# hmatuschek/libsdr

Measured on NVIDIA B200. Metric: iq_msamples_per_s_iqbaseband_fmdemod, higher is better.
Workload: dtype f32

## Files before the change

libsdr_b200/csrc/api.cu:

```cuda
#include "iqbb_kernels.cuh"

#include <atomic>
#include <cstdarg>
#include <cstdio>
#include <cmath>
#include <cstring>
#include <map>
#include <mutex>
#include <vector>

namespace sdrg {

static thread_local char g_err[512] = "";
static thread_local int g_device = 0;
static std::atomic<uint64_t> g_launches{0};

int set_error(int code, const char *fmt, ...) {
  va_list ap;
  va_start(ap, fmt);
  vsnprintf(g_err, sizeof(g_err), fmt, ap);
  va_end(ap);
  return code;
}
void count_launch(unsigned n) { g_launches.fetch_add(n, std::memory_order_relaxed); }
// ... 53 lines not shown

}

using namespace sdrg;

struct sdrg_iqbb {
  IqbbDesign d;
  int device = 0;
  bool configured = false;
  double nco_Fs = 0;
  void *d_taps = nullptr, *d_lut = nullptr;
  void *d_hist[2] = {nullptr, nullptr};
  void *d_acc[2] = {nullptr, nullptr};
  size_t acc_cap = 0;
  uint32_t acc_dirty[2] = {0, 0};
  uint32_t taps_len = 1, hist_len = 0;
  std::vector<int32_t> host_taps;
  int in_fmt = 0;
  bool real_input = false;
  double r_Ff = 0, r_width = 0, r_Fs = 0;
  int float_path = 0;
  bool fold = false;
  void *d_tab_a = nullptr, *d_tab_u = nullptr;
  void *d_tab_v = nullptr, *d_tab_cls = nullptr;
  uint32_t v_rows = 0, v_pitch = 0;
  int last_float_kernel = 0;
  uint32_t *d_work = nullptr;
  uint32_t phase0 = 0;
  int parity = 0;
  uint64_t consumed = 0, produced = 0;
// ... 174 lines not shown
int ensure_acc(sdrg_iqbb *h, size_t slots) {
  if (h->acc_cap >= slots) return SDRG_OK;
  const size_t cap = slots + slots / 2 + 64;
  void *n0 = nullptr, *n1 = nullptr;
  SDRG_CUDA(cudaMalloc(&n0, cap * acc_bytes()));
  SDRG_CUDA(cudaMalloc(&n1, cap * acc_bytes()));
  SDRG_CUDA(cudaMemset(n0, 0, cap * acc_bytes()));
  SDRG_CUDA(cudaMemset(n1, 0, cap * acc_bytes()));
  if (h->d_acc[0]) {
    SDRG_CUDA(cudaDeviceSynchronize());
    SDRG_CUDA(cudaMemcpy(h->parity == 0 ? n0 : n1, h->d_acc[h->parity], 2 * acc_bytes(), cudaMemcpyDeviceToDevice));
    cudaFree(h->d_acc[0]); cudaFree(h->d_acc[1]);
  }
  h->d_acc[0] = n0; h->d_acc[1] = n1;
  h->acc_dirty[0] = h->acc_dirty[1] = 0;
  h->acc_cap = cap;
  return SDRG_OK;
}

void reset_stream_state(sdrg_iqbb *h) {
  h->phase0 = 0; h->consumed = 0; h->produced = 0;
}

int design_only(sdrg_iqbb *h) {
  IqbbDesign &d = h->d;
  if (d.oFs > 0 && !h->real_input) {
    d.sub_sample = size_t(d.Fs / d.oFs);
    if (d.sub_sample < 1) d.sub_sample = 1;
  }
  if (d.sub_sample < 1) d.sub_sample = 1;
// ... 33 lines not shown
  const Advance adv = advance(h, n);
  *n_out = adv.n_out;
  int rc = ensure_acc(h, adv.n_out + 3);
  if (rc) return rc;
  const int p = h->parity, q = p ^ 1;
  IqbbAccumArgs a{};
  a.x = d_in; a.hist_in = h->d_hist[p]; a.hist_out = h->d_hist[q];
  a.taps = h->d_taps; a.lut = h->d_lut;
  a.host_taps = (h->d.scalar != SDRG_T_F32 && !h->host_taps.empty()) ? h->host_taps.data() : nullptr;
  a.acc_cur = h->d_acc[p]; a.acc_next = h->d_acc[q];
  a.n = n; a.taps_len = h->taps_len; a.hist_len = h->hist_len;
  a.ss = (uint32_t)h->d.sub_sample; a.r0 = adv.r0; a.first = adv.first;
  a.phase0 = h->phase0; a.inc = (uint32_t)(h->d.lut_inc & 0x7fffu); a.nco = h->d.lut_inc != 0 ? 1u : 0u;
  a.neg = h->d.negative ? 1u : 0u;
  a.zero_next = h->acc_dirty[q];
  a.in_fmt = (uint32_t)h->in_fmt;
  a.fir_shift = h->real_input ? (h->d.scalar == SDRG_T_S8 ? 8u : 16u) : 14u;
  IqbbFinalizeArgs f{};
  f.acc_cur = h->d_acc[p]; f.acc_next = h->d_acc[q];
  f.bb_out = d_bb; f.audio_out = d_audio;
  f.fm_last_in = fm_last_in; f.fm_last_out = fm_last_out;
  f.n_out = (uint32_t)adv.n_out; f.ss = a.ss; f.demod = (uint32_t)demod; f.e0 = adv.e0;
  f.seg = seg; f.in_place = (uint32_t)in_place;
  f.narrow16 = (h->real_input && h->d.scalar == SDRG_T_S8) ? 1u : 0u;
  if (h->fold) {
    IqbbFoldArgs fa{};
    fa.x = d_in; fa.acc_cur = a.acc_cur; fa.acc_next = a.acc_next;
    fa.tab_a = (const float2 *)h->d_tab_a; fa.tab_u = (const float2 *)h->d_tab_u;
    fa.tab_v = (const float2 *)h->d_tab_v; fa.tab_cls = (const uint16_t *)h->d_tab_cls;
    fa.v_rows = h->v_rows; fa.v_pitch = h->v_pitch;
    fa.n = n; fa.taps_len = (uint32_t)h->d.order; fa.ss = a.ss; fa.r0 = a.r0; fa.first = a.first;
    fa.phase0 = a.nco ? a.phase0 : 0u; fa.inc = a.nco ? a.inc : 0u;
    fa.zero_next = a.zero_next; fa.variant = h->float_path == 3 ? 2u : 0u;
    fa.work = h->d_work; f.work_reset = h->d_work;
    ProfScope ps(SDRG_KERNEL_IQBB_ACCUM, st);
    rc = launch_iqbb_fold(fa, st, &h->last_float_kernel);
  } else {
    ProfScope ps(SDRG_KERNEL_IQBB_ACCUM, st);
    if (h->d.scalar == SDRG_T_F32) h->last_float_kernel = 1;
    rc = launch_iqbb_accum(h->d.scalar, a, st);
  }
  if (rc) return rc;
  {
    ProfScope ps(SDRG_KERNEL_IQBB_FINALIZE, st);
    rc = launch_iqbb_finalize(h->d.scalar, f, st);
  }
  if (rc) return rc;
  h->acc_dirty[p] = (uint32_t)adv.n_out + 2;
  h->acc_dirty[q] = 2;
  h->parity = q;
  h->phase0 = (uint32_t)((h->phase0 + (uint64_t)n * (h->d.lut_inc & 0x7fffu)) & 0x7fffu);
  h->consumed += n; h->produced += adv.n_out;
  return SDRG_OK;
}

int check_handle(const sdrg_iqbb *h) {
  if (!h) return set_error(SDRG_ERR_ARG, "IQBaseBand: null handle");
  if (!h->configured) return set_error(SDRG_ERR_RUNTIME, "IQBaseBand: process() before config()");
  return SDRG_OK;
}

int config_common(const char *who, int expect_type, const sdrg_config *src, bool need_rate, bool *skip) {
  *skip = false;
  if (!src) return set_error(SDRG_ERR_ARG, "%s: null config", who);
// ... 287 lines not shown
  h->real_input = true; h->in_fmt = scalar == SDRG_T_S8 ? 5 : 4;
  h->r_Ff = Ff; h->r_width = width;
  return SDRG_OK;
}

int sdrg_iqbb_destroy(sdrg_iqbb *h) {
  if (!h) return SDRG_OK;
  cudaSetDevice(h->device);
  if (h->stream) { cudaStreamSynchronize(h->stream); cudaStreamDestroy(h->stream); }
  else cudaDeviceSynchronize();
  free_dev(&h->d_taps); free_dev(&h->d_lut);
  free_dev(&h->d_hist[0]); free_dev(&h->d_hist[1]);
  free_dev(&h->d_acc[0]); free_dev(&h->d_acc[1]);
  free_dev(&h->d_tab_a); free_dev(&h->d_tab_u); free_dev(&h->d_tab_v); free_dev(&h->d_tab_cls);
  if (h->d_work) { cudaFree(h->d_work); h->d_work = nullptr; }
  free_dev(&h->d_in); free_dev(&h->d_out);
  delete h;
  return SDRG_OK;
}

static int refresh_kernel(sdrg_iqbb *h) {
  if (!h->configured) return SDRG_OK;
  SDRG_CUDA(cudaSetDevice(h->device));
  SDRG_CUDA(cudaDeviceSynchronize());
  const uint32_t old_hist = h->hist_len;
  design_filter(h);
  std::vector<char> keep;
  const size_t sb = in_sample_bytes(h);
  if (old_hist) { keep.resize(old_hist * sb); SDRG_CUDA(cudaMemcpy(keep.data(), h->d_hist[h->parity], keep.size(), cudaMemcpyDeviceToHost)); }
  int rc = upload_design(h);
// ... 597 lines not shown
```

libsdr_b200/csrc/iqbb_finalize.cuh:

```cuda
#pragma once
#include "iqbb_kernels.cuh"
#include "demod_math.cuh"

namespace sdrg {

template <int SCALAR> struct Fin;
template <> struct Fin<SDRG_T_S16> {
  typedef int2 Acc; typedef short2 Bb; typedef short Fm; typedef short Au; typedef int Last;
  static __device__ __forceinline__ int2 value(const Acc s, uint32_t ss) {
    if (ss == 1) return make_int2((int)(short)s.x, (int)(short)s.y);
    return make_int2((int)(short)cdiv_component(s.x, (int)ss), (int)(short)cdiv_component(s.y, (int)ss));
  }
  static __device__ __forceinline__ Bb store(int2 v) { return make_short2((short)v.x, (short)v.y); }
  static __device__ __forceinline__ Last phi(int2 v) { return fm_phi_int(v.x, v.y); }
  static __device__ __forceinline__ Fm fm(Last last, Last p) { return (short)(last - p); }
  static __device__ __forceinline__ Fm fm_first(int2 v) { return (short)v.x; }
  static __device__ __forceinline__ Au am(int2 v) { return (short)am_int(v.x, v.y); }
  static __device__ __forceinline__ Au usb(int2 v) { return (short)usb_int(v.x, v.y); }
};
template <> struct Fin<SDRG_T_S8> {
  typedef int2 Acc; typedef char2 Bb; typedef short Fm; typedef signed char Au; typedef int Last;
  static __device__ __forceinline__ int2 value(const Acc s, uint32_t ss) {
    if (ss == 1) return make_int2((int)(signed char)s.x, (int)(signed char)s.y);
    return make_int2((int)(signed char)cdiv_component(s.x, (int)ss), (int)(signed char)cdiv_component(s.y, (int)ss));
// ... 32 lines not shown
}
template <int SCALAR>
__device__ __forceinline__ auto fin_value(const typename Fin<SCALAR>::Acc s, const IqbbFinalizeArgs &a) {
  if constexpr (SCALAR == SDRG_T_S8) { if (a.narrow16) return fin_value_s8_real(s, a.ss); }
  return Fin<SCALAR>::value(s, a.ss);
}

__device__ __forceinline__ bool seg_first(uint32_t j, const IqbbFinalizeArgs &a) {
  if (j == 0) return true;
  if (a.seg == 0) return false;
  const uint32_t e = a.e0 + j * a.ss;
  return (e % (uint32_t)a.seg) < a.ss;
}

template <int SCALAR>
__device__ __forceinline__ void iqbb_finalize_block(const IqbbFinalizeArgs &a, const uint32_t j0, const int tid,
                                                    typename Fin<SCALAR>::Last *sphi, unsigned char *sskip) {
  typedef Fin<SCALAR> F;
  const typename F::Acc *acc = (const typename F::Acc *)a.acc_cur;
  const uint32_t j = j0 + tid;
  const bool fm = a.demod == SDRG_DEMOD_FM;
  if (j == 0) {
    if (a.work_reset) *a.work_reset = 0u;
    ((typename F::Acc *)a.acc_next)[0] = acc[a.n_out];
    ((typename F::Acc *)a.acc_next)[1] = acc[a.n_out + 1];
    if (fm) {
      typename F::Last last = *(const typename F::Last *)a.fm_last_in;
      for (int64_t k = (int64_t)a.n_out - 1; k >= 0; --k) {
        if (!seg_first((uint32_t)k, a)) { last = F::phi(fin_value<SCALAR>(acc[k], a)); break; }
      }
      *(typename F::Last *)a.fm_last_out = last;
    }
  }
  const bool valid = j < a.n_out;
  auto v = fin_value<SCALAR>(valid ? acc[j] : typename F::Acc(), a);
  if (valid && a.bb_out) ((typename F::Bb *)a.bb_out)[j] = F::store(v);
  if (!a.audio_out) return;
  if (a.demod == SDRG_DEMOD_AM) { if (valid) ((typename F::Au *)a.audio_out)[j] = F::am(v); return; }
  if (a.demod == SDRG_DEMOD_USB) { if (valid) ((typename F::Au *)a.audio_out)[j] = F::usb(v); return; }
  if (!fm) return;
  const bool skip = !valid || seg_first(j, a);
  const typename F::Last p = skip ? typename F::Last(0) : F::phi(v);
  sphi[tid] = p; sskip[tid] = skip ? 1 : 0;
  __syncthreads();
  if (!valid) return;
  typename F::Fm *out = (typename F::Fm *)a.audio_out;
  if (skip) { if (a.in_place) out[j] = F::fm_first(v); return; }
  typename F::Last last;
  if (tid > 0 && !sskip[tid - 1]) last = sphi[tid - 1];
  else {
    int64_t k = (int64_t)j - 1;
    while (k >= 0 && seg_first((uint32_t)k, a)) --k;
    last = (k >= 0) ? F::phi(fin_value<SCALAR>(acc[k], a)) : *(const typename F::Last *)a.fm_last_in;
  }
  out[j] = F::fm(last, p);
}

}
```

libsdr_b200/csrc/iqbb_fold_kernels.cu:

```cuda
#include "iqbb_fold_common.cuh"

namespace sdrg {
using namespace foldk;
namespace {

template <int RS>
__device__ __forceinline__ void ragged_batch(float2 (&R)[8], const float2 *__restrict__ xk, uint32_t ph, uint32_t inc32,
                                             const float2 *sA, bool last_ok) {
  float2 xv[RS];
#pragma unroll
  for (int u = 0; u + 1 < RS; ++u) xv[u] = ld_stream(xk + 32 * u);
  xv[RS - 1] = make_float2(0.f, 0.f);
  if (last_ok) xv[RS - 1] = ld_stream(xk + 32 * (RS - 1));
#pragma unroll
  for (int u = 0; u < RS; ++u) cfma(R[u], sA[((ph + u * inc32) & 0x7fffu) >> 8], xv[u]);
}

__global__ void __launch_bounds__(kFoldThreads, 4) iqbb_fold_f32_kernel(const IqbbFoldArgs a) {
  extern __shared__ __align__(16) unsigned char dyn_smem[];
  __shared__ float2 sA[128];
  __shared__ float2 sH[256];
  const int tid = threadIdx.x, lane = tid & 31, warp = tid >> 5;

  for (uint32_t k = blockIdx.x * blockDim.x + tid; k < a.zero_next; k += gridDim.x * blockDim.x)
// ... 53 lines not shown
      cfma(sent, cmul(Ab, ut0), xt0);
      cfma(sent, cmul(Ab, ut1), xt1);
      float2 tot = make_float2(-sent.x, -sent.y);
#pragma unroll
      for (int u = 0; u < 8; ++u) cfma(tot, sH[(r0 + u * inc32) & 255u], R[u]);
      stage.push(tot, id, lane, acc_out);
      if (L1 > 0) stage.push(sent, id + 1, lane, acc_out);
      continue;
    }
    fold_chunk_general(a, id, total_warps, x, sA, sH, lane, L1, win_off, inc32, inc256, stage, acc_out);
  }
  stage.drain(lane, acc_out);

}

template <int S, int P = 0, int TS = 3>
__global__ void __launch_bounds__(kFoldThreads, S <= 8 ? 4 : (S <= 13 ? 3 : 2)) iqbb_fold_f32_win_kernel(const IqbbFoldArgs a) {
  extern __shared__ __align__(16) unsigned char dyn_smem[];
  __shared__ float2 sA[128];
  __shared__ float2 sH[256];
  const int tid = threadIdx.x, lane = tid & 31, warp = tid >> 5;
  for (uint32_t k = blockIdx.x * blockDim.x + tid; k < a.zero_next; k += gridDim.x * blockDim.x)
    ((float2 *)a.acc_next)[k] = make_float2(0.f, 0.f);
  if (tid < 128) sA[tid] = a.tab_a[tid];
  sH[tid] = a.tab_u[(size_t)tid * a.taps_len];
  __syncthreads();

  const uint32_t T = gridDim.x * kFoldWarps;
  const uint32_t wg = warp * gridDim.x + blockIdx.x;
  const float2 *__restrict__ x = (const float2 *)a.x;
  float *acc_out = (float *)a.acc_cur;
  WarpStage stage{(float2 *)dyn_smem + (size_t)warp * kStageRows * kStagePitch, 0u, 0u};
  const int L1 = (int)a.taps_len - 1;
  const int win_off = (int)a.first - (int)a.r0;
  const uint32_t inc32 = (32u * a.inc) & 0x7fffu, inc256 = (256u * a.inc) & 0x7fffu;
  const bool last_ok = (uint32_t)lane < a.fast_pl;
  int te[TS]; bool te_ok[TS];
#pragma unroll
  for (int k = 0; k < TS; ++k) { te[k] = (int)a.ss - 32 * (S - 1 - k) - lane; te_ok[k] = te[k] >= 1 && te[k] <= L1; }

  if (wg == 0) fold_chunk_general(a, 0u, T, x, sA, sH, lane, L1, win_off, inc32, inc256, stage, acc_out);
  else if (a.fast_hi + wg < a.n_chunks) fold_chunk_general(a, a.fast_hi + wg, T, x, sA, sH, lane, L1, win_off, inc32, inc256, stage, acc_out);
  const uint32_t kWorkChunk = a.work_chunk;
  const uint32_t n_work = (a.fast_hi + kWorkChunk - 1) / kWorkChunk;
  uint32_t grabbed = 0;
  if (lane == 0) grabbed = atomicAdd(a.work, 1u);
  const uint32_t c0 = __shfl_sync(kFull, grabbed, 0);
  if (c0 < n_work) {
    uint32_t id = 1 + c0 * kWorkChunk, end = min(id + kWorkChunk, a.fast_hi + 1);
    if (lane == 0) grabbed = atomicAdd(a.work, 1u);
    const float2 *__restrict__ xc = x + ((int)(id * a.ss) + win_off) + lane;
    float2 ring[S];
#pragma unroll
    for (int i = 0; i + 1 < S; ++i) ring[i] = ld_stream(xc + 32 * i);
    ring[S - 1] = make_float2(0.f, 0.f);
    if (last_ok) ring[S - 1] = ld_stream(xc + 32 * (S - 1));
    float2 carry = make_float2(0.f, 0.f);
    for (;;) {
      uint32_t nid = id + 1;
      bool more = nid < end, switched = false;
      if (!more) {
        const uint32_t cn = __shfl_sync(kFull, grabbed, 0);
        if (cn < n_work) { nid = 1 + cn * kWorkChunk; more = true; switched = true; }
      }
// ... 20 lines not shown
        if (!(P & 1) && S - 1 - i < TS) cfma(ts, ut[S - 1 - i], ring[i]);
        if (more) {
          if (i + 1 < S) ring[i] = ld_stream(xn + 32 * i);
          else if (last_ok) ring[i] = ld_stream(xn + 32 * i);
        }
      }
      const float2 sent = cmul(Ab, ts);
      float2 tot = make_float2(-sent.x, -sent.y);
      const uint32_t r0 = ph & 255u;
#pragma unroll
      for (int u = 0; u < 8; ++u) {
        if (P & 4) { tot.x += R[u].x; tot.y += R[u].y; }
        else cfma(tot, sH[(r0 + u * inc32) & 255u], R[u]);
      }
      tot.x += carry.x; tot.y += carry.y;
      stage.push(tot, id, lane, acc_out);
      carry = sent;
      if ((!more || switched) && L1 > 0 && !(P & 1)) { stage.push(carry, id + 1, lane, acc_out); carry = make_float2(0.f, 0.f); }
      if (!more) break;
      if (switched) {
        end = min(nid + kWorkChunk, a.fast_hi + 1);
        if (lane == 0) grabbed = atomicAdd(a.work, 1u);
      }
      id = nid;
    }
  }
  stage.drain(lane, acc_out);
}

template <int S, int P = 0, int TS = 3>
static int launch_fold_win_s(const IqbbFoldArgs &a, cudaStream_t st) {
  static std::atomic<int> resident_dev[kMaxDevices];
  const size_t smem = (size_t)kFoldWarps * kStageRows * kStagePitch * sizeof(float2);
  const int dev = current_device();
  if (!resident_dev[dev]) {
    SDRG_CUDA(cudaFuncSetAttribute(iqbb_fold_f32_win_kernel<S, P, TS>, cudaFuncAttributeMaxDynamicSharedMemorySize, (int)smem));
    int sms = 0, per_sm = 0;
    SDRG_CUDA(cudaDeviceGetAttribute(&sms, cudaDevAttrMultiProcessorCount, dev));
    SDRG_CUDA(cudaOccupancyMaxActiveBlocksPerMultiprocessor(&per_sm, iqbb_fold_f32_win_kernel<S, P, TS>, kFoldThreads, smem));
    resident_dev[dev] = sms * (per_sm > 0 ? per_sm : 1);
  }
  const uint64_t resident = (uint64_t)resident_dev[dev];
  const uint64_t want = ((uint64_t)a.n_chunks + kFoldWarps - 1) / kFoldWarps;
  iqbb_fold_f32_win_kernel<S, P, TS><<<(unsigned)(want < resident ? want : resident), kFoldThreads, smem, st>>>(a);
  SDRG_CHECK_LAUNCH("iqbb_fold_f32_win_kernel");
  return SDRG_OK;
}

static int launch_fold_win(const IqbbFoldArgs &a, cudaStream_t st) {
#ifdef SDRG_EXPERIMENTS
  static const int wp = env_int("SDRG_FOLD_WINP", 0);
  if (wp && (a.ss + 31) / 32 == 13) {
    switch (wp) {
      case 1: return launch_fold_win_s<13, 1>(a, st); case 2: return launch_fold_win_s<13, 2>(a, st);
      case 3: return launch_fold_win_s<13, 3>(a, st); case 4: return launch_fold_win_s<13, 4>(a, st);
      case 5: return launch_fold_win_s<13, 5>(a, st); case 6: return launch_fold_win_s<13, 6>(a, st);
      case 7: return launch_fold_win_s<13, 7>(a, st); case 8: return launch_fold_win_s<13, 8>(a, st); default: break;
    }
  }
#endif
  if (a.taps_len > 65) {
    switch ((a.ss + 31) / 32) {
      case 3: return launch_fold_win_s<3, 0, 5>(a, st);   case 4: return launch_fold_win_s<4, 0, 5>(a, st);
      case 5: return launch_fold_win_s<5, 0, 5>(a, st);   case 6: return launch_fold_win_s<6, 0, 5>(a, st);
      case 7: return launch_fold_win_s<7, 0, 5>(a, st);   case 8: return launch_fold_win_s<8, 0, 5>(a, st);
      case 9: return launch_fold_win_s<9, 0, 5>(a, st);   case 10: return launch_fold_win_s<10, 0, 5>(a, st);
      case 11: return launch_fold_win_s<11, 0, 5>(a, st); case 12: return launch_fold_win_s<12, 0, 5>(a, st);
      case 13: return launch_fold_win_s<13, 0, 5>(a, st); case 14: return launch_fold_win_s<14, 0, 5>(a, st);
      case 15: return launch_fold_win_s<15, 0, 5>(a, st); case 16: return launch_fold_win_s<16, 0, 5>(a, st);
      default: return set_error(SDRG_ERR_RUNTIME, "IQBaseBand<float>: window-pipelined kernel needs 65 <= sub_sample <= 512 for more than 65 taps");
    }
  }
  switch ((a.ss + 31) / 32) {
    case 1: return launch_fold_win_s<1>(a, st);   case 2: return launch_fold_win_s<2>(a, st);
    case 3: return launch_fold_win_s<3>(a, st);   case 4: return launch_fold_win_s<4>(a, st);
    case 5: return launch_fold_win_s<5>(a, st);   case 6: return launch_fold_win_s<6>(a, st);
    case 7: return launch_fold_win_s<7>(a, st);   case 8: return launch_fold_win_s<8>(a, st);
    case 9: return launch_fold_win_s<9>(a, st);   case 10: return launch_fold_win_s<10>(a, st);
    case 11: return launch_fold_win_s<11>(a, st); case 12: return launch_fold_win_s<12>(a, st);
    case 13: return launch_fold_win_s<13>(a, st); case 14: return launch_fold_win_s<14>(a, st);
    case 15: return launch_fold_win_s<15>(a, st); case 16: return launch_fold_win_s<16>(a, st);
    default: return set_error(SDRG_ERR_RUNTIME, "IQBaseBand<float>: window-pipelined kernel needs sub_sample <= 512");
  }
}

constexpr int kSmallTile = 2048;

__global__ void __launch_bounds__(kFoldThreads, 4) iqbb_fold_f32_small_kernel(const IqbbFoldArgs a) {
  extern __shared__ __align__(16) unsigned char dyn_smem[];
  __shared__ float2 sA[128];
  __shared__ float2 sH[256];
  float2 *zo = (float2 *)dyn_smem, *zn = zo + kSmallTile;
  const int tid = threadIdx.x;
  for (uint32_t k = blockIdx.x * blockDim.x + tid; k < a.zero_next; k += gridDim.x * blockDim.x)
    ((float2 *)a.acc_next)[k] = make_float2(0.f, 0.f);
  if (tid < 128) sA[tid] = a.tab_a[tid];
// ... 83 lines not shown
  const int dev = current_device();
  if (!resident_dev[dev]) {
    SDRG_CUDA(cudaFuncSetAttribute(iqbb_fold_f32_small_kernel, cudaFuncAttributeMaxDynamicSharedMemorySize, (int)smem));
    int sms = 0, per_sm = 0;
    SDRG_CUDA(cudaDeviceGetAttribute(&sms, cudaDevAttrMultiProcessorCount, dev));
    SDRG_CUDA(cudaOccupancyMaxActiveBlocksPerMultiprocessor(&per_sm, iqbb_fold_f32_small_kernel, kFoldThreads, smem));
    resident_dev[dev] = sms * (per_sm > 0 ? per_sm : 1);
  }
  const uint64_t n_tiles = ((uint64_t)a.n + kSmallTile - 1) / kSmallTile;
  const uint64_t resident = (uint64_t)resident_dev[dev];
  iqbb_fold_f32_small_kernel<<<(unsigned)(n_tiles < resident ? n_tiles : resident), kFoldThreads, smem, st>>>(a);
  SDRG_CHECK_LAUNCH("iqbb_fold_f32_small_kernel");
  return SDRG_OK;
}

}

static int launch_fold_ldg(IqbbFoldArgs a, cudaStream_t st, int *which) {
  const uint64_t q_last = (uint64_t)a.r0 + (a.n - 1) - ((a.first && a.n > 1) ? 1 : 0);
  const uint64_t n_slots = q_last / a.ss + 1;
  a.part = 8192;
  a.cpw = (uint32_t)(((uint64_t)a.ss + 1 + a.part - 1) / a.part);
  const uint64_t n_chunks = n_slots * a.cpw;
  if (n_chunks > 0xffffffffull) return set_error(SDRG_ERR_RUNTIME, "IQBaseBand<float>: too many windows in one call");
  a.n_chunks = (uint32_t)n_chunks;
  a.chunks_per_warp = 0;
  static const int pf = env_int("SDRG_FOLD_PF", 0);
  a.pf_dist = (uint32_t)pf;
  static const int fast_env = env_int("SDRG_FOLD_FAST", 1);
  a.fast = (fast_env && a.cpw == 1 && a.taps_len <= 65 && a.ss + 1 >= a.taps_len) ? 1u : 0u;
  const bool win_ok = fast_env && a.cpw == 1 && a.taps_len <= 129 && a.ss + 1 >= a.taps_len && a.ss <= 512;
  a.fast_nb = a.ss / 256;
  a.fast_rs = (a.ss % 256 + 31) / 32;
// ... 3 lines not shown
    const int64_t hi = ((int64_t)a.n + (int64_t)a.r0 - (int64_t)a.first) / (int64_t)a.ss - 1;
    a.fast_hi = hi >= 1 ? (uint32_t)hi : 0u;
  }
  static const int win_env = env_int("SDRG_FOLD_WIN", 1);
  static const int chunk_env = env_int("SDRG_FOLD_WORK_CHUNK", 16);
  a.work_chunk = (uint32_t)(chunk_env > 0 ? chunk_env : 16);
#ifdef SDRG_EXPERIMENTS
  static const int probe = env_int("SDRG_FOLD_PROBE", 0);
#else
  constexpr int probe = 0;
#endif
  static const int perwin_max = env_int("SDRG_FOLD_PERWIN_MAX", 256);
  if (!probe && a.cpw == 1 && (int)a.ss <= perwin_max && fold_perwin_eligible(a)) { *which = 5; return launch_fold_perwin(a, st); }
  static const int small_env = env_int("SDRG_FOLD_SMALL", 55);
  if (!probe && a.cpw == 1 && a.ss + 1 >= a.taps_len && (a.ss < 32 || (int)a.ss <= small_env)) { *which = 4; return launch_fold_small(a, st); }
  if (!probe && win_env && win_ok && a.fast_hi >= 1) { *which = 3; return launch_fold_win(a, st); }
#ifdef SDRG_EXPERIMENTS
  if (probe >= 1 && probe <= 3) return launch_fold_probe(probe, a, st);
#endif
  static std::atomic<int> resident_dev[kMaxDevices];
  const size_t smem = (size_t)kFoldWarps * kStageRows * kStagePitch * sizeof(float2);
  const int dev = current_device();
  if (!resident_dev[dev]) {
    SDRG_CUDA(cudaFuncSetAttribute(iqbb_fold_f32_kernel, cudaFuncAttributeMaxDynamicSharedMemorySize, (int)smem));
    int sms = 0, per_sm = 0;
    SDRG_CUDA(cudaDeviceGetAttribute(&sms, cudaDevAttrMultiProcessorCount, dev));
    SDRG_CUDA(cudaOccupancyMaxActiveBlocksPerMultiprocessor(&per_sm, iqbb_fold_f32_kernel, kFoldThreads, smem));
    resident_dev[dev] = sms * (per_sm > 0 ? per_sm : 1);
  }
  *which = 2;
  const int resident = resident_dev[dev];
  const uint64_t want = (n_chunks + kFoldWarps - 1) / kFoldWarps;
  const unsigned grid = (unsigned)(want < (uint64_t)resident ? want : (uint64_t)resident);
  iqbb_fold_f32_kernel<<<grid, kFoldThreads, smem, st>>>(a);
  SDRG_CHECK_LAUNCH("iqbb_fold_f32_kernel");
  return SDRG_OK;
}

int launch_iqbb_fold(const IqbbFoldArgs &a, cudaStream_t st, int *which_out) {
  int which_local = 0;
  int *which = which_out ? which_out : &which_local;
  if (a.n == 0) return SDRG_OK;
  const bool aligned = (reinterpret_cast<uintptr_t>(a.x) & 15u) == 0;
#ifdef SDRG_EXPERIMENTS
  static const int env_variant = env_int("SDRG_FOLD_VARIANT", 0);
  const int variant = a.variant ? (int)a.variant : env_variant;
  if (aligned && variant == 2 && a.ss >= 32) { *which = 6; return launch_fold_tma(a, st); }
#else
  (void)aligned;
#endif
  return launch_fold_ldg(a, st, which);
}

}
```

libsdr_b200/csrc/iqbb_kernels.cuh:

```cuda
#pragma once
#include "common.cuh"

namespace sdrg {

constexpr int kIqbbThreads = 256;
constexpr int kIqbbPerThread = 8;
constexpr int kIqbbTile = kIqbbThreads * kIqbbPerThread;

struct IqbbAccumArgs {
  const void *x;
  const void *hist_in;
  void       *hist_out;
  const void *taps;
  const void *host_taps;
  const void *lut;
  void       *acc_cur;
  void       *acc_next;
  uint32_t    n;
  uint32_t    taps_len;
  uint32_t    hist_len;
  uint32_t    ss;
  uint32_t    r0;
  uint32_t    first;
  uint32_t    phase0;
  uint32_t    inc;
  uint32_t    nco;
  uint32_t    neg;
  uint32_t    zero_next;
  uint32_t    in_fmt;
  uint32_t    fir_shift;
  uint32_t    div_m, div_s;
  uint32_t    zero;
};

struct IqbbFoldArgs {
  const void   *x;
  void         *acc_cur;
  void         *acc_next;
  const float2 *tab_a;
  const float2 *tab_u;
  uint32_t      n;
  uint32_t      taps_len;
  uint32_t      ss;
  uint32_t      r0, first;
  uint32_t      phase0, inc;
  uint32_t      zero_next;
  uint32_t      part;
  uint32_t      cpw;
  uint32_t      n_chunks;
  uint32_t      chunks_per_warp;
  uint32_t      pf_dist;
  uint32_t      seg;
  uint32_t      variant;
  uint32_t      fast;
  uint32_t      fast_nb;
  uint32_t      fast_rs;
  uint32_t      fast_pl;
  uint32_t      fast_hi;
  uint32_t     *work;
  uint32_t      work_chunk;
  const float2 *tab_v;
  const uint16_t *tab_cls;
  uint32_t      v_rows, v_pitch;
  uint32_t      d_lo, d_hi;
};

struct IqbbFinalizeArgs {
  uint32_t   *work_reset;
  const void *acc_cur;
  void       *acc_next;
  void       *bb_out;
  void       *audio_out;
  const void *fm_last_in;
  void       *fm_last_out;
  uint32_t    n_out;
  uint32_t    ss;
  uint32_t    demod;
  uint32_t    e0;
  uint64_t    seg;
  uint32_t    in_place;
  uint32_t    narrow16;
};

struct BankAccumArgs {
  const void     *x, *hist_in;
  void           *hist_out;
  const void     *taps;
  const void     *lut;
  const void     *tab_u;
  const uint32_t *inc;
  const uint32_t *neg;
  void           *acc_cur, *acc_next;
  size_t          acc_stride;
  uint32_t        n, channels, group, taps_len, hist_len, ss, r0, first;
  uint32_t        consumed15;
  uint32_t        zero_next;
};
struct BankFinalizeStrides { size_t acc_stride, out_stride; uint32_t bb_bytes, audio_bytes; };

int launch_iqbb_accum(int scalar, const IqbbAccumArgs &a, cudaStream_t st);
int launch_bank_accum(int scalar, const BankAccumArgs &a, cudaStream_t st);
int launch_bank_finalize(int scalar, const IqbbFinalizeArgs &a, const BankFinalizeStrides &s, uint32_t channels, cudaStream_t st);
int launch_iqbb_finalize(int scalar, const IqbbFinalizeArgs &a, cudaStream_t st);
int launch_iqbb_fold(const IqbbFoldArgs &a, cudaStream_t st, int *which = nullptr);

int launch_fmdemod(int scalar, const void *in, size_t n, void *out, const void *last_in, void *last_out,
                   int in_place, cudaStream_t st);
int launch_amdemod(int scalar, const void *in, size_t n, void *out, cudaStream_t st);
int launch_usbdemod(int scalar, const void *in, size_t n, void *out, cudaStream_t st);
int launch_autocast_cs16(int fmt, const void *in, size_t n_bytes, void *out, cudaStream_t st);
int launch_autocast(int kind, const void *in, size_t n_scalars, void *out, cudaStream_t st);
int launch_fmdeemph(const void *in, void *out, size_t n, size_t streams, size_t stride, int alpha, void *avg, cudaStream_t st);

}
```

Baseline: 785,000.

## Fuse finalize and FM demod into window-pipelined fold kernel via mailbox boundaries

Work chunks of the window fold kernel now finalize their own output windows in-kernel: each warp sums its staged rows, computes baseband values, phases and FM demod output directly. Adjacent chunks exchange boundary partial sums and phases through a per-chunk mailbox with atomic handshakes. A small edge kernel then handles only the first and last windows instead of a full finalize pass. The zeroing of the next accumulator is also restricted to the range the fused path does not already cover. This removes the separate finalize kernel's read of the accumulator buffer and a full launch, at the cost of added cross-block synchronization, extra shared memory per warp, and more register pressure in the hot kernel.

```diff
diff --git a/libsdr_b200/csrc/api.cu b/libsdr_b200/csrc/api.cu
--- a/libsdr_b200/csrc/api.cu
+++ b/libsdr_b200/csrc/api.cu
@@ -91,6 +91,9 @@
   void *d_acc[2] = {nullptr, nullptr};
   size_t acc_cap = 0;
   uint32_t acc_dirty[2] = {0, 0};
+  uint32_t acc_dirty_lo[2] = {0, 0};
+  FoldMbox *d_mbox = nullptr;
+  uint32_t mbox_cap = 0;
   uint32_t taps_len = 1, hist_len = 0;
   std::vector<int32_t> host_taps;
   int in_fmt = 0;
@@ -295,6 +298,12 @@
   }
   h->d_acc[0] = n0; h->d_acc[1] = n1;
   h->acc_dirty[0] = h->acc_dirty[1] = 0;
+  h->acc_dirty_lo[0] = h->acc_dirty_lo[1] = 0;
+  if (h->d_mbox) { cudaFree(h->d_mbox); h->d_mbox = nullptr; h->mbox_cap = 0; }
+  const size_t mb = cap / kFoldMboxWindows + 2;
+  SDRG_CUDA(cudaMalloc((void **)&h->d_mbox, mb * sizeof(FoldMbox)));
+  SDRG_CUDA(cudaMemset(h->d_mbox, 0, mb * sizeof(FoldMbox)));
+  h->mbox_cap = (uint32_t)mb;
   h->acc_cap = cap;
   return SDRG_OK;
 }
@@ -358,6 +367,7 @@
   a.phase0 = h->phase0; a.inc = (uint32_t)(h->d.lut_inc & 0x7fffu); a.nco = h->d.lut_inc != 0 ? 1u : 0u;
   a.neg = h->d.negative ? 1u : 0u;
   a.zero_next = h->acc_dirty[q];
+  const uint32_t zero_lo = h->acc_dirty_lo[q];
   a.in_fmt = (uint32_t)h->in_fmt;
   a.fir_shift = h->real_input ? (h->d.scalar == SDRG_T_S8 ? 8u : 16u) : 14u;
   IqbbFinalizeArgs f{};
@@ -367,6 +377,7 @@
   f.n_out = (uint32_t)adv.n_out; f.ss = a.ss; f.demod = (uint32_t)demod; f.e0 = adv.e0;
   f.seg = seg; f.in_place = (uint32_t)in_place;
   f.narrow16 = (h->real_input && h->d.scalar == SDRG_T_S8) ? 1u : 0u;
+  uint32_t n_fused = 0;
   if (h->fold) {
     IqbbFoldArgs fa{};
     fa.x = d_in; fa.acc_cur = a.acc_cur; fa.acc_next = a.acc_next;
@@ -375,10 +386,11 @@
     fa.v_rows = h->v_rows; fa.v_pitch = h->v_pitch;
     fa.n = n; fa.taps_len = (uint32_t)h->d.order; fa.ss = a.ss; fa.r0 = a.r0; fa.first = a.first;
     fa.phase0 = a.nco ? a.phase0 : 0u; fa.inc = a.nco ? a.inc : 0u;
-    fa.zero_next = a.zero_next; fa.variant = h->float_path == 3 ? 2u : 0u;
+    fa.zero_next = a.zero_next; fa.zero_lo = zero_lo; fa.variant = h->float_path == 3 ? 2u : 0u;
     fa.work = h->d_work; f.work_reset = h->d_work;
+    fa.mbox = h->d_mbox; fa.mbox_cap = h->mbox_cap;
     ProfScope ps(SDRG_KERNEL_IQBB_ACCUM, st);
-    rc = launch_iqbb_fold(fa, st, &h->last_float_kernel);
+    rc = launch_iqbb_fold(fa, st, &h->last_float_kernel, &f, &n_fused);
   } else {
     ProfScope ps(SDRG_KERNEL_IQBB_ACCUM, st);
     if (h->d.scalar == SDRG_T_F32) h->last_float_kernel = 1;
@@ -387,11 +399,13 @@
   if (rc) return rc;
   {
     ProfScope ps(SDRG_KERNEL_IQBB_FINALIZE, st);
-    rc = launch_iqbb_finalize(h->d.scalar, f, st);
+    rc = n_fused ? launch_fold_edge(f, h->d_mbox, n_fused, st) : launch_iqbb_finalize(h->d.scalar, f, st);
   }
   if (rc) return rc;
   h->acc_dirty[p] = (uint32_t)adv.n_out + 2;
+  h->acc_dirty_lo[p] = n_fused ? 1 + n_fused * kFoldMboxWindows : 0;
   h->acc_dirty[q] = 2;
+  h->acc_dirty_lo[q] = 0;
   h->parity = q;
   h->phase0 = (uint32_t)((h->phase0 + (uint64_t)n * (h->d.lut_inc & 0x7fffu)) & 0x7fffu);
   h->consumed += n; h->produced += adv.n_out;
@@ -709,6 +723,7 @@
   free_dev(&h->d_acc[0]); free_dev(&h->d_acc[1]);
   free_dev(&h->d_tab_a); free_dev(&h->d_tab_u); free_dev(&h->d_tab_v); free_dev(&h->d_tab_cls);
   if (h->d_work) { cudaFree(h->d_work); h->d_work = nullptr; }
+  if (h->d_mbox) { cudaFree(h->d_mbox); h->d_mbox = nullptr; }
   free_dev(&h->d_in); free_dev(&h->d_out);
   delete h;
   return SDRG_OK;
diff --git a/libsdr_b200/csrc/iqbb_finalize.cuh b/libsdr_b200/csrc/iqbb_finalize.cuh
--- a/libsdr_b200/csrc/iqbb_finalize.cuh
+++ b/libsdr_b200/csrc/iqbb_finalize.cuh
@@ -70,24 +70,33 @@
 }
 
 template <int SCALAR>
+__device__ __forceinline__ typename Fin<SCALAR>::Last last_before(const IqbbFinalizeArgs &a, const uint32_t j) {
+  typedef Fin<SCALAR> F;
+  const typename F::Acc *acc = (const typename F::Acc *)a.acc_cur;
+  int64_t k = (int64_t)j - 1;
+  while (k >= (int64_t)a.k_lo && seg_first((uint32_t)k, a)) --k;
+  if (k >= (int64_t)a.k_lo) return F::phi(fin_value<SCALAR>(acc[k], a));
+  return *(const typename F::Last *)(a.k_lo ? a.fm_last_mid : a.fm_last_in);
+}
+
+template <int SCALAR>
+__device__ __forceinline__ void finalize_carry(const IqbbFinalizeArgs &a) {
+  typedef Fin<SCALAR> F;
+  const typename F::Acc *acc = (const typename F::Acc *)a.acc_cur;
+  if (a.work_reset) *a.work_reset = 0u;
+  ((typename F::Acc *)a.acc_next)[0] = acc[a.n_out];
+  ((typename F::Acc *)a.acc_next)[1] = acc[a.n_out + 1];
+  if (a.demod == SDRG_DEMOD_FM) *(typename F::Last *)a.fm_last_out = last_before<SCALAR>(a, a.n_out);
+}
+
+template <int SCALAR>
 __device__ __forceinline__ void iqbb_finalize_block(const IqbbFinalizeArgs &a, const uint32_t j0, const int tid,
                                                     typename Fin<SCALAR>::Last *sphi, unsigned char *sskip) {
   typedef Fin<SCALAR> F;
   const typename F::Acc *acc = (const typename F::Acc *)a.acc_cur;
   const uint32_t j = j0 + tid;
   const bool fm = a.demod == SDRG_DEMOD_FM;
-  if (j == 0) {
-    if (a.work_reset) *a.work_reset = 0u;
-    ((typename F::Acc *)a.acc_next)[0] = acc[a.n_out];
-    ((typename F::Acc *)a.acc_next)[1] = acc[a.n_out + 1];
-    if (fm) {
-      typename F::Last last = *(const typename F::Last *)a.fm_last_in;
-      for (int64_t k = (int64_t)a.n_out - 1; k >= 0; --k) {
-        if (!seg_first((uint32_t)k, a)) { last = F::phi(fin_value<SCALAR>(acc[k], a)); break; }
-      }
-      *(typename F::Last *)a.fm_last_out = last;
-    }
-  }
+  if (j == 0) finalize_carry<SCALAR>(a);
   const bool valid = j < a.n_out;
   auto v = fin_value<SCALAR>(valid ? acc[j] : typename F::Acc(), a);
   if (valid && a.bb_out) ((typename F::Bb *)a.bb_out)[j] = F::store(v);
@@ -102,14 +111,21 @@
   if (!valid) return;
   typename F::Fm *out = (typename F::Fm *)a.audio_out;
   if (skip) { if (a.in_place) out[j] = F::fm_first(v); return; }
-  typename F::Last last;
-  if (tid > 0 && !sskip[tid - 1]) last = sphi[tid - 1];
-  else {
-    int64_t k = (int64_t)j - 1;
-    while (k >= 0 && seg_first((uint32_t)k, a)) --k;
-    last = (k >= 0) ? F::phi(fin_value<SCALAR>(acc[k], a)) : *(const typename F::Last *)a.fm_last_in;
-  }
+  const typename F::Last last = (tid > 0 && !sskip[tid - 1]) ? sphi[tid - 1] : last_before<SCALAR>(a, j);
   out[j] = F::fm(last, p);
 }
 
+__device__ __forceinline__ void fin_emit_f32(const IqbbFinalizeArgs &a, const uint32_t j, const float2 v, const bool skip,
+                                             const bool has_last, const double last, const double p) {
+  typedef Fin<SDRG_T_F32> F;
+  if (a.bb_out) ((F::Bb *)a.bb_out)[j] = F::store(v);
+  if (!a.audio_out) return;
+  if (a.demod == SDRG_DEMOD_AM) { ((F::Au *)a.audio_out)[j] = F::am(v); return; }
+  if (a.demod == SDRG_DEMOD_USB) { ((F::Au *)a.audio_out)[j] = F::usb(v); return; }
+  if (a.demod != SDRG_DEMOD_FM) return;
+  F::Fm *out = (F::Fm *)a.audio_out;
+  if (skip) { if (a.in_place) out[j] = F::fm_first(v); return; }
+  if (has_last) out[j] = F::fm(last, p);
 }
+
+}
diff --git a/libsdr_b200/csrc/iqbb_fold_kernels.cu b/libsdr_b200/csrc/iqbb_fold_kernels.cu
--- a/libsdr_b200/csrc/iqbb_fold_kernels.cu
+++ b/libsdr_b200/csrc/iqbb_fold_kernels.cu
@@ -1,4 +1,5 @@
 #include "iqbb_fold_common.cuh"
+#include "iqbb_finalize.cuh"
 
 namespace sdrg {
 using namespace foldk;
@@ -91,14 +92,93 @@
 
 }
 
-template <int S, int P = 0, int TS = 3>
-__global__ void __launch_bounds__(kFoldThreads, S <= 8 ? 4 : (S <= 13 ? 3 : 2)) iqbb_fold_f32_win_kernel(const IqbbFoldArgs a) {
+
+__device__ __forceinline__ void fold_complete_boundary(const IqbbFinalizeArgs &f, const uint32_t b, const float2 s0, const float2 t,
+                                                       const double phi1, const double phi2, const double lprev) {
+  typedef Fin<SDRG_T_F32> F;
+  const float2 v = F::value(make_float2(s0.x + t.x, s0.y + t.y), f.ss);
+  const bool fm = f.demod == SDRG_DEMOD_FM;
+  const bool skip0 = fm && seg_first(b, f);
+  const double p0 = (fm && !skip0) ? F::phi(v) : 0.0;
+  fin_emit_f32(f, b, v, skip0, true, lprev, p0);
+  if (!fm || !f.audio_out) return;
+  const double last0 = skip0 ? lprev : p0;
+  F::Fm *out = (F::Fm *)f.audio_out;
+  if (!seg_first(b + 1, f)) out[b + 1] = F::fm(last0, phi1);
+  else out[b + 2] = F::fm(last0, phi2);
+}
+
+__device__ __forceinline__ float2 ld_volatile(const float2 *p) {
+  return make_float2(*(const volatile float *)&p->x, *(const volatile float *)&p->y);
+}
+__device__ __forceinline__ double ld_volatile(const double *p) { return *(const volatile double *)p; }
+
+__device__ __forceinline__ void fold_fused_drain(const IqbbFoldArgs &a, const IqbbFinalizeArgs &f, const float2 *rows, const int lane,
+                                                 const uint32_t b, const uint32_t c, float *acc_out) {
+  typedef Fin<SDRG_T_F32> F;
+  __syncwarp();
+  float sr = 0.f, si = 0.f;
+  if (lane <= kStageRows) {
+    const float2 *r = rows + lane * kStagePitch;
+#pragma unroll 8
+    for (int i = 0; i < 32; ++i) { const float2 v = r[i]; sr += v.x; si += v.y; }
+  }
+  __syncwarp();
+  const uint32_t j = b + (uint32_t)lane;
+  const bool win = lane >= 1 && lane < kStageRows;
+  const float2 v = F::value(make_float2(sr, si), a.ss);
+  const bool fm = f.demod == SDRG_DEMOD_FM;
+  const bool skip = fm && lane < kStageRows && seg_first(j, f);
+  const double p = (fm && win && !skip) ? F::phi(v) : 0.0;
+  const uint32_t skipm = __ballot_sync(kFull, skip);
+  const double p1 = __shfl_up_sync(kFull, p, 1), p2 = __shfl_up_sync(kFull, p, 2);
+  if (win) {
+    const bool prev_skip = (skipm >> (lane - 1)) & 1u;
+    fin_emit_f32(f, j, v, skip, prev_skip ? lane >= 3 : lane >= 2, prev_skip ? p2 : p1, p);
+  }
+  const double phi1 = __shfl_sync(kFull, p, 1), phi2 = __shfl_sync(kFull, p, 2);
+  const double lend = __shfl_sync(kFull, p, ((skipm >> (kStageRows - 1)) & 1u) ? kStageRows - 2 : kStageRows - 1);
+  const float2 t = make_float2(__shfl_sync(kFull, sr, kStageRows), __shfl_sync(kFull, si, kStageRows));
+  if (lane != 0) return;
+  FoldMbox *mb = a.mbox;
+  if (c + 1 < a.n_fused) {
+    FoldMbox *m = mb + c + 1;
+    m->t = t; m->lprev = lend;
+    __threadfence();
+    if (atomicAdd(&m->count, 1u) == 1u) {
+      __threadfence();
+      fold_complete_boundary(f, b + kStageRows, ld_volatile(&m->s0), t, ld_volatile(&m->phi1), ld_volatile(&m->phi2), lend);
+      m->count = 0u;
+    }
+  } else {
+    if (t.x != 0.f || t.y != 0.f) { atomicAdd(acc_out + 2 * (size_t)(b + kStageRows), t.x); atomicAdd(acc_out + 2 * (size_t)(b + kStageRows) + 1, t.y); }
+    mb[a.n_fused].lprev = lend;
+  }
+  FoldMbox *m = mb + c;
+  m->s0 = make_float2(sr, si); m->phi1 = phi1; m->phi2 = phi2;
+  __threadfence();
+  if (atomicAdd(&m->count, 1u) == 1u) {
+    __threadfence();
+    fold_complete_boundary(f, b, make_float2(sr, si), ld_volatile(&m->t), phi1, phi2, ld_volatile(&m->lprev));
+    m->count = 0u;
+  }
+}
+
+constexpr int kWinStageRows = kStageRows + 1;
+static_assert(kStageRows == (int)kFoldMboxWindows, "a finalizing chunk is one stage of windows");
+
+template <int S, int P = 0, int TS = 3, bool FUSE = false>
+__global__ void __launch_bounds__(kFoldThreads, S <= 8 ? 4 : (S <= 13 ? 3 : 2)) iqbb_fold_f32_win_kernel(const IqbbFoldArgs a, const IqbbFinalizeArgs f) {
   extern __shared__ __align__(16) unsigned char dyn_smem[];
   __shared__ float2 sA[128];
   __shared__ float2 sH[256];
   const int tid = threadIdx.x, lane = tid & 31, warp = tid >> 5;
-  for (uint32_t k = blockIdx.x * blockDim.x + tid; k < a.zero_next; k += gridDim.x * blockDim.x)
-    ((float2 *)a.acc_next)[k] = make_float2(0.f, 0.f);
+  {
+    const uint32_t z2 = min(a.zero_next, 2u), zlo = max(a.zero_lo, 2u);
+    const uint32_t nz = z2 + (a.zero_next > zlo ? a.zero_next - zlo : 0u);
+    for (uint32_t k = blockIdx.x * blockDim.x + tid; k < nz; k += gridDim.x * blockDim.x)
+      ((float2 *)a.acc_next)[k < z2 ? k : zlo + (k - z2)] = make_float2(0.f, 0.f);
+  }
   if (tid < 128) sA[tid] = a.tab_a[tid];
   sH[tid] = a.tab_u[(size_t)tid * a.taps_len];
   __syncthreads();
@@ -107,7 +187,7 @@
   const uint32_t wg = warp * gridDim.x + blockIdx.x;
   const float2 *__restrict__ x = (const float2 *)a.x;
   float *acc_out = (float *)a.acc_cur;
-  WarpStage stage{(float2 *)dyn_smem + (size_t)warp * kStageRows * kStagePitch, 0u, 0u};
+  WarpStage stage{(float2 *)dyn_smem + (size_t)warp * kWinStageRows * kStagePitch, 0u, 0u};
   const int L1 = (int)a.taps_len - 1;
   const int win_off = (int)a.first - (int)a.r0;
   const uint32_t inc32 = (32u * a.inc) & 0x7fffu, inc256 = (256u * a.inc) & 0x7fffu;
@@ -118,13 +198,14 @@
 
   if (wg == 0) fold_chunk_general(a, 0u, T, x, sA, sH, lane, L1, win_off, inc32, inc256, stage, acc_out);
   else if (a.fast_hi + wg < a.n_chunks) fold_chunk_general(a, a.fast_hi + wg, T, x, sA, sH, lane, L1, win_off, inc32, inc256, stage, acc_out);
+  if (FUSE) stage.drain(lane, acc_out);
   const uint32_t kWorkChunk = a.work_chunk;
   const uint32_t n_work = (a.fast_hi + kWorkChunk - 1) / kWorkChunk;
   uint32_t grabbed = 0;
   if (lane == 0) grabbed = atomicAdd(a.work, 1u);
   const uint32_t c0 = __shfl_sync(kFull, grabbed, 0);
   if (c0 < n_work) {
-    uint32_t id = 1 + c0 * kWorkChunk, end = min(id + kWorkChunk, a.fast_hi + 1);
+    uint32_t c = c0, id = 1 + c0 * kWorkChunk, end = min(id + kWorkChunk, a.fast_hi + 1);
     if (lane == 0) grabbed = atomicAdd(a.work, 1u);
     const float2 *__restrict__ xc = x + ((int)(id * a.ss) + win_off) + lane;
     float2 ring[S];
@@ -175,11 +256,22 @@
         else cfma(tot, sH[(r0 + u * inc32) & 255u], R[u]);
       }
       tot.x += carry.x; tot.y += carry.y;
-      stage.push(tot, id, lane, acc_out);
-      carry = sent;
-      if ((!more || switched) && L1 > 0 && !(P & 1)) { stage.push(carry, id + 1, lane, acc_out); carry = make_float2(0.f, 0.f); }
+      const bool fused = FUSE && c < a.n_fused;
+      if (fused) {
+        const uint32_t b = 1 + c * kWorkChunk;
+        stage.rows[(id - b) * kStagePitch + lane] = tot;
+        if (id + 1 == end) {
+          stage.rows[kStageRows * kStagePitch + lane] = sent;
+          fold_fused_drain(a, f, stage.rows, lane, b, c, acc_out);
+        }
+      } else {
+        stage.push(tot, id, lane, acc_out);
+      }
+      carry = (fused && id + 1 == end) ? make_float2(0.f, 0.f) : sent;
+      if (!fused && (!more || switched) && L1 > 0 && !(P & 1)) { stage.push(carry, id + 1, lane, acc_out); carry = make_float2(0.f, 0.f); }
       if (!more) break;
       if (switched) {
+        c = __shfl_sync(kFull, grabbed, 0);
         end = min(nid + kWorkChunk, a.fast_hi + 1);
         if (lane == 0) grabbed = atomicAdd(a.work, 1u);
       }
@@ -189,58 +281,64 @@
   stage.drain(lane, acc_out);
 }
 
-template <int S, int P = 0, int TS = 3>
-static int launch_fold_win_s(const IqbbFoldArgs &a, cudaStream_t st) {
+template <int S, int P, int TS, bool FUSE>
+static int launch_fold_win_f(const IqbbFoldArgs &a, const IqbbFinalizeArgs &f, cudaStream_t st) {
   static std::atomic<int> resident_dev[kMaxDevices];
-  const size_t smem = (size_t)kFoldWarps * kStageRows * kStagePitch * sizeof(float2);
+  const size_t smem = (size_t)kFoldWarps * kWinStageRows * kStagePitch * sizeof(float2);
   const int dev = current_device();
   if (!resident_dev[dev]) {
-    SDRG_CUDA(cudaFuncSetAttribute(iqbb_fold_f32_win_kernel<S, P, TS>, cudaFuncAttributeMaxDynamicSharedMemorySize, (int)smem));
+    SDRG_CUDA(cudaFuncSetAttribute(iqbb_fold_f32_win_kernel<S, P, TS, FUSE>, cudaFuncAttributeMaxDynamicSharedMemorySize, (int)smem));
     int sms = 0, per_sm = 0;
     SDRG_CUDA(cudaDeviceGetAttribute(&sms, cudaDevAttrMultiProcessorCount, dev));
-    SDRG_CUDA(cudaOccupancyMaxActiveBlocksPerMultiprocessor(&per_sm, iqbb_fold_f32_win_kernel<S, P, TS>, kFoldThreads, smem));
+    SDRG_CUDA(cudaOccupancyMaxActiveBlocksPerMultiprocessor(&per_sm, iqbb_fold_f32_win_kernel<S, P, TS, FUSE>, kFoldThreads, smem));
     resident_dev[dev] = sms * (per_sm > 0 ? per_sm : 1);
   }
   const uint64_t resident = (uint64_t)resident_dev[dev];
   const uint64_t want = ((uint64_t)a.n_chunks + kFoldWarps - 1) / kFoldWarps;
-  iqbb_fold_f32_win_kernel<S, P, TS><<<(unsigned)(want < resident ? want : resident), kFoldThreads, smem, st>>>(a);
+  iqbb_fold_f32_win_kernel<S, P, TS, FUSE><<<(unsigned)(want < resident ? want : resident), kFoldThreads, smem, st>>>(a, f);
   SDRG_CHECK_LAUNCH("iqbb_fold_f32_win_kernel");
   return SDRG_OK;
 }
 
-static int launch_fold_win(const IqbbFoldArgs &a, cudaStream_t st) {
+template <int S, int P = 0, int TS = 3>
+static int launch_fold_win_s(const IqbbFoldArgs &a, const IqbbFinalizeArgs &f, cudaStream_t st) {
+  if (a.n_fused) return launch_fold_win_f<S, P, TS, true>(a, f, st);
+  return launch_fold_win_f<S, P, TS, false>(a, f, st);
+}
+
+static int launch_fold_win(const IqbbFoldArgs &a, const IqbbFinalizeArgs &f, cudaStream_t st) {
 #ifdef SDRG_EXPERIMENTS
   static const int wp = env_int("SDRG_FOLD_WINP", 0);
   if (wp && (a.ss + 31) / 32 == 13) {
     switch (wp) {
-      case 1: return launch_fold_win_s<13, 1>(a, st); case 2: return launch_fold_win_s<13, 2>(a, st);
-      case 3: return launch_fold_win_s<13, 3>(a, st); case 4: return launch_fold_win_s<13, 4>(a, st);
-      case 5: return launch_fold_win_s<13, 5>(a, st); case 6: return launch_fold_win_s<13, 6>(a, st);
-      case 7: return launch_fold_win_s<13, 7>(a, st); case 8: return launch_fold_win_s<13, 8>(a, st); default: break;
+      case 1: return launch_fold_win_s<13, 1>(a, f, st); case 2: return launch_fold_win_s<13, 2>(a, f, st);
+      case 3: return launch_fold_win_s<13, 3>(a, f, st); case 4: return launch_fold_win_s<13, 4>(a, f, st);
+      case 5: return launch_fold_win_s<13, 5>(a, f, st); case 6: return launch_fold_win_s<13, 6>(a, f, st);
+      case 7: return launch_fold_win_s<13, 7>(a, f, st); case 8: return launch_fold_win_s<13, 8>(a, f, st); default: break;
     }
   }
 #endif
   if (a.taps_len > 65) {
     switch ((a.ss + 31) / 32) {
-      case 3: return launch_fold_win_s<3, 0, 5>(a, st);   case 4: return launch_fold_win_s<4, 0, 5>(a, st);
-      case 5: return launch_fold_win_s<5, 0, 5>(a, st);   case 6: return launch_fold_win_s<6, 0, 5>(a, st);
-      case 7: return launch_fold_win_s<7, 0, 5>(a, st);   case 8: return launch_fold_win_s<8, 0, 5>(a, st);
-      case 9: return launch_fold_win_s<9, 0, 5>(a, st);   case 10: return launch_fold_win_s<10, 0, 5>(a, st);
-      case 11: return launch_fold_win_s<11, 0, 5>(a, st); case 12: return launch_fold_win_s<12, 0, 5>(a, st);
-      case 13: return launch_fold_win_s<13, 0, 5>(a, st); case 14: return launch_fold_win_s<14, 0, 5>(a, st);
-      case 15: return launch_fold_win_s<15, 0, 5>(a, st); case 16: return launch_fold_win_s<16, 0, 5>(a, st);
+      case 3: return launch_fold_win_s<3, 0, 5>(a, f, st);   case 4: return launch_fold_win_s<4, 0, 5>(a, f, st);
+      case 5: return launch_fold_win_s<5, 0, 5>(a, f, st);   case 6: return launch_fold_win_s<6, 0, 5>(a, f, st);
+      case 7: return launch_fold_win_s<7, 0, 5>(a, f, st);   case 8: return launch_fold_win_s<8, 0, 5>(a, f, st);
+      case 9: return launch_fold_win_s<9, 0, 5>(a, f, st);   case 10: return launch_fold_win_s<10, 0, 5>(a, f, st);
+      case 11: return launch_fold_win_s<11, 0, 5>(a, f, st); case 12: return launch_fold_win_s<12, 0, 5>(a, f, st);
+      case 13: return launch_fold_win_s<13, 0, 5>(a, f, st); case 14: return launch_fold_win_s<14, 0, 5>(a, f, st);
+      case 15: return launch_fold_win_s<15, 0, 5>(a, f, st); case 16: return launch_fold_win_s<16, 0, 5>(a, f, st);
       default: return set_error(SDRG_ERR_RUNTIME, "IQBaseBand<float>: window-pipelined kernel needs 65 <= sub_sample <= 512 for more than 65 taps");
     }
   }
   switch ((a.ss + 31) / 32) {
-    case 1: return launch_fold_win_s<1>(a, st);   case 2: return launch_fold_win_s<2>(a, st);
-    case 3: return launch_fold_win_s<3>(a, st);   case 4: return launch_fold_win_s<4>(a, st);
-    case 5: return launch_fold_win_s<5>(a, st);   case 6: return launch_fold_win_s<6>(a, st);
-    case 7: return launch_fold_win_s<7>(a, st);   case 8: return launch_fold_win_s<8>(a, st);
-    case 9: return launch_fold_win_s<9>(a, st);   case 10: return launch_fold_win_s<10>(a, st);
-    case 11: return launch_fold_win_s<11>(a, st); case 12: return launch_fold_win_s<12>(a, st);
-    case 13: return launch_fold_win_s<13>(a, st); case 14: return launch_fold_win_s<14>(a, st);
-    case 15: return launch_fold_win_s<15>(a, st); case 16: return launch_fold_win_s<16>(a, st);
+    case 1: return launch_fold_win_s<1>(a, f, st);   case 2: return launch_fold_win_s<2>(a, f, st);
+    case 3: return launch_fold_win_s<3>(a, f, st);   case 4: return launch_fold_win_s<4>(a, f, st);
+    case 5: return launch_fold_win_s<5>(a, f, st);   case 6: return launch_fold_win_s<6>(a, f, st);
+    case 7: return launch_fold_win_s<7>(a, f, st);   case 8: return launch_fold_win_s<8>(a, f, st);
+    case 9: return launch_fold_win_s<9>(a, f, st);   case 10: return launch_fold_win_s<10>(a, f, st);
+    case 11: return launch_fold_win_s<11>(a, f, st); case 12: return launch_fold_win_s<12>(a, f, st);
+    case 13: return launch_fold_win_s<13>(a, f, st); case 14: return launch_fold_win_s<14>(a, f, st);
+    case 15: return launch_fold_win_s<15>(a, f, st); case 16: return launch_fold_win_s<16>(a, f, st);
     default: return set_error(SDRG_ERR_RUNTIME, "IQBaseBand<float>: window-pipelined kernel needs sub_sample <= 512");
   }
 }
@@ -354,9 +452,35 @@
   return SDRG_OK;
 }
 
-}
-
-static int launch_fold_ldg(IqbbFoldArgs a, cudaStream_t st, int *which) {
+__global__ void __launch_bounds__(256) iqbb_fold_edge_kernel(IqbbFinalizeArgs f, FoldMbox *mbox, const uint32_t n_fused) {
+  __shared__ double sphi[256];
+  __shared__ unsigned char sskip[256];
+  typedef Fin<SDRG_T_F32> F;
+  const float2 *acc = (const float2 *)f.acc_cur;
+  const uint32_t b_last = 1 + n_fused * kStageRows;
+  f.k_lo = b_last;
+  f.fm_last_mid = &mbox[n_fused].lprev;
+  if (blockIdx.x > 0) { iqbb_finalize_block<SDRG_T_F32>(f, b_last + (blockIdx.x - 1) * 256u, (int)threadIdx.x, sphi, sskip); return; }
+  if (threadIdx.x == 0) finalize_carry<SDRG_T_F32>(f);
+  if (threadIdx.x == 1) fin_emit_f32(f, 0, F::value(acc[0], f.ss), true, false, 0.0, 0.0);
+  if (threadIdx.x == 2) {
+    const double lprev = f.demod == SDRG_DEMOD_FM ? *(const double *)f.fm_last_in : 0.0;
+    fold_complete_boundary(f, 1, mbox[0].s0, acc[1], mbox[0].phi1, mbox[0].phi2, lprev);
+    mbox[0].count = 0u;
+  }
+}
+
+}
+
+int launch_fold_edge(const IqbbFinalizeArgs &f, FoldMbox *mbox, uint32_t n_fused, cudaStream_t st) {
+  const uint32_t b_last = 1 + n_fused * kStageRows;
+  const unsigned grid = 1 + (f.n_out > b_last ? (f.n_out - b_last + 255) / 256 : 0);
+  iqbb_fold_edge_kernel<<<grid, 256, 0, st>>>(f, mbox, n_fused);
+  SDRG_CHECK_LAUNCH("iqbb_fold_edge_kernel");
+  return SDRG_OK;
+}
+
+static int launch_fold_ldg(IqbbFoldArgs a, cudaStream_t st, int *which, const IqbbFinalizeArgs *fin, uint32_t *n_fused) {
   const uint64_t q_last = (uint64_t)a.r0 + (a.n - 1) - ((a.first && a.n > 1) ? 1 : 0);
   const uint64_t n_slots = q_last / a.ss + 1;
   a.part = 8192;
@@ -390,7 +514,17 @@
   if (!probe && a.cpw == 1 && (int)a.ss <= perwin_max && fold_perwin_eligible(a)) { *which = 5; return launch_fold_perwin(a, st); }
   static const int small_env = env_int("SDRG_FOLD_SMALL", 55);
   if (!probe && a.cpw == 1 && a.ss + 1 >= a.taps_len && (a.ss < 32 || (int)a.ss <= small_env)) { *which = 4; return launch_fold_small(a, st); }
-  if (!probe && win_env && win_ok && a.fast_hi >= 1) { *which = 3; return launch_fold_win(a, st); }
+  if (!probe && win_env && win_ok && a.fast_hi >= 1) {
+    *which = 3;
+    const uint32_t n_work = (a.fast_hi + a.work_chunk - 1) / a.work_chunk;
+    static const int fuse_env = env_int("SDRG_FOLD_FUSE", 1);
+    a.n_fused = 0;
+    if (fuse_env && fin && n_fused && a.mbox && a.work_chunk == (uint32_t)kStageRows && n_work >= 2 && n_work <= a.mbox_cap &&
+        (fin->seg == 0 || fin->seg >= 2 * (uint64_t)a.ss + 2))
+      a.n_fused = n_work - 1;
+    if (n_fused) *n_fused = a.n_fused;
+    return launch_fold_win(a, fin ? *fin : IqbbFinalizeArgs{}, st);
+  }
 #ifdef SDRG_EXPERIMENTS
   if (probe >= 1 && probe <= 3) return launch_fold_probe(probe, a, st);
 #endif
@@ -413,9 +547,10 @@
   return SDRG_OK;
 }
 
-int launch_iqbb_fold(const IqbbFoldArgs &a, cudaStream_t st, int *which_out) {
+int launch_iqbb_fold(const IqbbFoldArgs &a, cudaStream_t st, int *which_out, const IqbbFinalizeArgs *fin, uint32_t *n_fused) {
   int which_local = 0;
   int *which = which_out ? which_out : &which_local;
+  if (n_fused) *n_fused = 0;
   if (a.n == 0) return SDRG_OK;
   const bool aligned = (reinterpret_cast<uintptr_t>(a.x) & 15u) == 0;
 #ifdef SDRG_EXPERIMENTS
@@ -425,7 +560,7 @@
 #else
   (void)aligned;
 #endif
-  return launch_fold_ldg(a, st, which);
-}
-
-}
+  return launch_fold_ldg(a, st, which, fin, n_fused);
+}
+
+}
diff --git a/libsdr_b200/csrc/iqbb_kernels.cuh b/libsdr_b200/csrc/iqbb_kernels.cuh
--- a/libsdr_b200/csrc/iqbb_kernels.cuh
+++ b/libsdr_b200/csrc/iqbb_kernels.cuh
@@ -33,6 +33,8 @@
   uint32_t    zero;
 };
 
+struct FoldMbox;
+
 struct IqbbFoldArgs {
   const void   *x;
   void         *acc_cur;
@@ -63,6 +65,18 @@
   const uint16_t *tab_cls;
   uint32_t      v_rows, v_pitch;
   uint32_t      d_lo, d_hi;
+  uint32_t      zero_lo;
+  FoldMbox     *mbox;
+  uint32_t      mbox_cap;
+  uint32_t      n_fused;
+};
+
+constexpr uint32_t kFoldMboxWindows = 16;
+struct FoldMbox {
+  float2   s0, t;
+  double   phi1, phi2, lprev;
+  uint32_t count;
+  uint32_t pad;
 };
 
 struct IqbbFinalizeArgs {
@@ -80,6 +94,8 @@
   uint64_t    seg;
   uint32_t    in_place;
   uint32_t    narrow16;
+  uint32_t    k_lo;
+  const void *fm_last_mid;
 };
 
 struct BankAccumArgs {
@@ -102,7 +118,9 @@
 int launch_bank_accum(int scalar, const BankAccumArgs &a, cudaStream_t st);
 int launch_bank_finalize(int scalar, const IqbbFinalizeArgs &a, const BankFinalizeStrides &s, uint32_t channels, cudaStream_t st);
 int launch_iqbb_finalize(int scalar, const IqbbFinalizeArgs &a, cudaStream_t st);
-int launch_iqbb_fold(const IqbbFoldArgs &a, cudaStream_t st, int *which = nullptr);
+int launch_iqbb_fold(const IqbbFoldArgs &a, cudaStream_t st, int *which = nullptr, const IqbbFinalizeArgs *fin = nullptr,
+                     uint32_t *n_fused = nullptr);
+int launch_fold_edge(const IqbbFinalizeArgs &f, FoldMbox *mbox, uint32_t n_fused, cudaStream_t st);
 
 int launch_fmdemod(int scalar, const void *in, size_t n, void *out, const void *last_in, void *last_out,
                    int in_place, cudaStream_t st);
diff --git a/scratch/fold_win_sass.py b/scratch/fold_win_sass.py
--- /dev/null
+++ b/scratch/fold_win_sass.py
@@ -0,0 +1,55 @@
+import argparse
+import collections
+import os
+import re
+import subprocess
+import tempfile
+
+ROOT = os.path.join(os.path.dirname(os.path.abspath(__file__)), "..")
+SRC = os.path.join(ROOT, "libsdr_b200", "csrc", "iqbb_fold_kernels.cu")
+NVCC = os.environ.get("NVCC", "/usr/local/cuda/bin/nvcc")
+CUOBJDUMP = os.path.join(os.path.dirname(NVCC), "cuobjdump")
+
+
+def main():
+    ap = argparse.ArgumentParser()
+    ap.add_argument("--s", type=int, default=13)
+    ap.add_argument("--ts", type=int, default=3)
+    ap.add_argument("--fuse", type=int, default=1)
+    args = ap.parse_args()
+    tag = "iqbb_fold_f32_win_kernelILi%dELi0ELi%dELb%dE" % (args.s, args.ts, args.fuse)
+    with tempfile.TemporaryDirectory() as tmp:
+        cubin = os.path.join(tmp, "fold.cubin")
+        r = subprocess.run([NVCC, "-gencode", "arch=compute_100a,code=sm_100a", "-O3", "-std=c++17", "-cubin",
+                            "-Xptxas", "-v", SRC, "-o", cubin], capture_output=True, text=True, check=True)
+        info = r.stderr.splitlines()
+        for i, line in enumerate(info):
+            if tag in line:
+                print("\n".join(l.strip() for l in info[i + 1:i + 3]))
+                break
+        sass = subprocess.run([CUOBJDUMP, "-sass", cubin], capture_output=True, text=True, check=True).stdout
+    funcs = re.split(r"\n\s*Function : ", sass)
+    body = next(f for f in funcs if tag in f.split("\n", 1)[0])
+    ins = []
+    for line in body.splitlines():
+        m = re.match(r"\s*/\*([0-9a-f]+)\*/\s+(@!?U?P\w+\s+)?([A-Z][A-Z0-9_.]*)([^;]*);", line)
+        if m:
+            ins.append((int(m.group(1), 16), m.group(3), m.group(4)))
+    at = {a: k for k, (a, _, _) in enumerate(ins)}
+    best = None
+    for k, (a, op, rest) in enumerate(ins):
+        t = re.match(r"\s*(0x[0-9a-f]+)", rest)
+        if op == "BRA" and t and int(t.group(1), 16) <= a and int(t.group(1), 16) in at:
+            lo = at[int(t.group(1), 16)]
+            n_ffma2 = sum(1 for _, o, _ in ins[lo:k + 1] if o.startswith("FFMA2"))
+            if best is None or n_ffma2 > best[0]:
+                best = (n_ffma2, lo, k)
+    _, lo, hi = best
+    hist = collections.Counter(o.split(".")[0] for _, o, _ in ins[lo:hi + 1])
+    print("%s: window loop = %d static instructions" % (tag, hi - lo + 1))
+    for op, n in hist.most_common():
+        print("  %-8s %d" % (op, n))
+
+
+if __name__ == "__main__":
+    main()
```

Result: slower. 713,900 (median of 6 runs) (-9.1%).
